# eth-cscs/conflux

Hardware: NVIDIA H100
Metric: LU GFLOP/s (FP64, (2/3)N^3) (higher is better)
Workload: dtype f64

## Files before the change

### conflux_b200/csrc/kernels.h

```cpp
#pragma once
#include <cuda_runtime.h>

#include <cstdint>
#include <memory>

#include "common.cuh"

namespace cflx {

struct GemmArgs {
    int M, N, K;
    const double* AT;
    int64_t ldat;
    const double* B;
    int64_t ldb;
    const double* C;
    int64_t ldc;
    double* D;
    int64_t ldd;
    double alpha, beta;
};
int gemm_tn_setup();
int launch_gemm_tn(const GemmArgs& g, cudaStream_t stream);

struct OzakiWorkspace {
    struct Maps;
    DevBuf<int8_t> planesA;
    DevBuf<int8_t> planesB;
    DevBuf<int> ea;
    DevBuf<int> eb;
    std::unique_ptr<Maps> maps;
    int K = 0, cap_a = 0, cap_b = 0, sms = 0;
    OzakiWorkspace();
    ~OzakiWorkspace();
};
int ozaki_workspace_create(OzakiWorkspace* ws, int max_rows, int max_cols, int K);
int ozaki_split_a(OzakiWorkspace* ws, const double* LT, int64_t ld, int n, cudaStream_t s);
int ozaki_split_b(OzakiWorkspace* ws, const double* U, int64_t ld, int col0, int n, cudaStream_t s);
int wgmma_peak_probe(int n, double* tmacs_out);
int launch_ozaki_gemm(OzakiWorkspace* ws, int M, int N, int row0, int col0, double* C, int64_t ldc, int max_ctas, cudaStream_t s);

struct PanelWorkspace {
    DevBuf<uint2> slot_hdr;
    DevBuf<uint2> slot_rows;
    int epoch;
    int max_ctas;
    int cta_cap;
    DevBuf<unsigned> sk_flags;
    DevBuf<int> sk_ppos;
    DevBuf<unsigned> sk_ticket;
    unsigned sk_epoch, sk_ticket_count;
    int sk_enabled;
};
int panel_workspace_create(PanelWorkspace* ws);
int launch_panel_getrf(double* W, int64_t ldw, int n, int v, int* perm_out, PanelWorkspace* ws, cudaStream_t stream);
int launch_panel_getrf_a00(double* W, int64_t ldw, int n, int v, int* perm_out, double* A00, int* nb_used,
                           PanelWorkspace* ws, cudaStream_t stream);

int launch_extract_panel_T(const double* A, int64_t lda, int64_t row0, int64_t col0, int n, int v, double* PT,
                           int64_t ldp, cudaStream_t stream);
int launch_store_panel_T(double* A, int64_t lda, int64_t row0, int64_t col0, int n, int v, const double* LT,
                         int64_t ldp, cudaStream_t stream);
int launch_gather_winners(const double* PT, int64_t ldp, const int* tags, int n_valid, const int* perm, int v,
                          double* out_vals, int64_t ldo, int* out_tags, int dst0, cudaStream_t stream);
int launch_gather_a00(const double* W, int64_t ldw, const int* perm, int v, int nb, double* A00, double* A00T,
                      cudaStream_t stream);

struct MovePlan {
    int* npiv;
    int* cur_piv;
    int* order;
    int* slot2piv;
    int* early;
    int* late;
    int* nel;
    int* rowsrc;
};
int launch_plan_moves(const int* gpivots, int v, int Px, int pi, int fnpr, int Ml, const int* igri, MovePlan plan,
                      cudaStream_t stream);
int launch_push_phase1(const double* A, int64_t lda, int ncols, int col_lo, MovePlan plan, int v, double* tmp,
                       double* a01raw, int64_t ld01, int c0, cudaStream_t stream);
int launch_push_phase2(double* A, int64_t lda, int ncols, int col_lo, MovePlan plan, int v, cudaStream_t stream);
int launch_push_phase3(double* A, int64_t lda, int ncols, int col_lo, int fnpr, MovePlan plan, int v,
                       const double* tmp, cudaStream_t stream);
int launch_update_gri(int* gri, int* gri_tmp, int* igri, const int* rowsrc, int fnpr, int Ml, int v, int Px,
                      cudaStream_t stream);
int launch_compact_panel(const double* PT, int64_t ldp, double* PT2, int64_t ldp2, const int* rowsrc, int fnpr_old,
                         const int* npiv, int Ml, int v, cudaStream_t stream);
int launch_store_u_rows(double* A, int64_t lda, int fnpr_old, MovePlan plan, const double* U, int64_t ldu, int c0,
                        int ncols, int v, cudaStream_t stream);
int launch_store_diag(double* A, int64_t lda, int fnpr_old, MovePlan plan, const double* A00, int loff, int v,
                      cudaStream_t stream);
int launch_split_factors(const double* F, int64_t ldf, int n, double* LT, double* U, cudaStream_t stream);
int launch_gather_perm_rows(const double* A, int64_t lda, const int* perm, int n, double* out, cudaStream_t stream);
constexpr int SUMSQ_PARTIALS = 1184;
int launch_sumsq(const double* X, int64_t count, double* out, double* partials, cudaStream_t stream);
int launch_sum_partials(const double* partials, int n, double* out, cudaStream_t stream);
int launch_fill(double* p, int64_t n, double val, cudaStream_t stream);
int launch_iota_gri(int* gri, int* igri, int Ml, int v, int Px, int pi, cudaStream_t stream);
int launch_pack_bcast(const double* A00, const int* tags, int v, double* buf, cudaStream_t stream);
int launch_unpack_bcast(const double* buf, int v, double* A00, double* A00T, int* gpivots, cudaStream_t stream);
int launch_record_pivots(const int* gpivots, int v, int* hist, int k, cudaStream_t stream);

int launch_diag_inverses(const double* A00, int v, int nb, double* Uinv, double* LinvT, cudaStream_t stream);
int trsm_right_upper_T(const double* A00, const double* Uinv, int v, int nb, double* PT, double* LT, int64_t ld,
                       int n, cudaStream_t stream);
int trsm_left_lower_unit(const double* A00T, const double* LinvT, int v, int nb, double* R, double* U, int64_t ld,
                         int n, cudaStream_t stream);

size_t potrf_tile_scratch(int v);
int potrf_setup(int v);
int potrf_tile(double* D, double* UT, double* Q, int* info, int col0, int v, cudaStream_t stream, int64_t* launches);
int potrf_block128(double* D, int ldd, double* UT, int ldu, double* Uc, int* info, int col0, cudaStream_t stream);

bool getrf_nopiv_blocked(int v);
size_t getrf_nopiv_scratch(int v, bool blocked);
int launch_getrf_nopiv_tile(const double* Bt, int v, double tiny, double* A, double* AT, const int* tags_in, int* tags_out,
                            int* rec, int col0, bool blocked, double* scratch, cudaStream_t stream, int64_t* launches);
int launch_fixed_locate(const int* rows, int v, int Px, int pi, int fnpr, int n_old, const int* igri, int* pos,
                        cudaStream_t stream);
int launch_fixed_info_operand(int* rec, cudaStream_t stream);

int launch_gather_rows(const double* A, int64_t lda, const int* src_rows, int nrows, int ncols, double* out,
                       cudaStream_t stream);

int launch_gemm_narrow(int M, int N, int K, const double* A, int64_t lda, const double* B, int64_t ldb, const double* C,
                       int64_t ldc, double* D, int64_t ldd, double alpha, double beta, cudaStream_t stream);
int launch_gemm_narrow_tn(int M, int N, int K, const double* AT, int64_t ldat, const double* B, int64_t ldb,
                          const double* C, int64_t ldc, double* D, int64_t ldd, double alpha, double beta,
                          cudaStream_t stream);

enum class ResidMode { NN, TN, SymLower };

}
```

### conflux_b200/csrc/panel.cu

```cuda
#include <cooperative_groups.h>

#include <climits>
#include <cstdlib>

#include "common.cuh"
#include "kernels.h"

namespace cflx {

namespace {
constexpr int PT_THREADS = 256;
constexpr int PT_WARPS = PT_THREADS / 32;
constexpr int PT_LAUNCH = PT_THREADS + 32;
constexpr int PT_ALLWARPS = PT_LAUNCH / 32;
constexpr int MAXG = 132;
constexpr int RPT_LIMIT = 8;

struct PanelArgs {
    double* W;
    int64_t ldw;
    int n, v, nsteps;
    int R, Rpad, G;
    int* perm_out;
    double* A00;
    uint2* slot_hdr;
    uint2* slot_rows;
    int epoch_base;
};

__device__ __forceinline__ void st_ll(uint2* p, unsigned data, unsigned epoch) {
    asm volatile("st.volatile.global.v2.u32 [%0], {%1, %2};" ::"l"(p), "r"(data), "r"(epoch) : "memory");
}
__device__ __forceinline__ uint4 ld_ll2(const uint2* p) {
    uint4 v;
    asm volatile("ld.volatile.global.v4.u32 {%0, %1, %2, %3}, [%4];" : "=r"(v.x), "=r"(v.y), "=r"(v.z), "=r"(v.w) : "l"(p) : "memory");
    return v;
}

struct Cand {
    unsigned long long key;
    int pos;
    int row;
};

__device__ __forceinline__ Cand warp_argmax(Cand c) {
    const unsigned hi = (unsigned)(c.key >> 32), lo = (unsigned)c.key;
    const unsigned m1 = __reduce_max_sync(0xffffffffu, hi);
    bool in = (hi == m1);
    const unsigned m2 = __reduce_max_sync(0xffffffffu, in ? lo : 0u);
    in = in && (lo == m2);
    const unsigned m3 = __reduce_min_sync(0xffffffffu, in ? (unsigned)c.pos : (unsigned)INT_MAX);
    const unsigned ballot = __ballot_sync(0xffffffffu, in && (unsigned)c.pos == m3);
    const int src = __ffs(ballot) - 1;
    Cand r;
    r.key = ((unsigned long long)m1 << 32) | m2;
    r.pos = (int)m3;
    r.row = __shfl_sync(0xffffffffu, c.row, src);
    return r;
}
__device__ __forceinline__ bool better(const Cand& a, const Cand& b) {
    return a.key > b.key || (a.key == b.key && a.pos < b.pos);
}
__device__ __forceinline__ Cand block_argmax(Cand c, unsigned long long* red_key, int* red_pos, int* red_row, int& rb) {
    Cand w = warp_argmax(c);
    const int warp = threadIdx.x >> 5, lane = threadIdx.x & 31;
    const int o = rb * PT_ALLWARPS;
    rb ^= 1;
    if (lane == 0) {
        red_key[o + warp] = w.key;
        red_pos[o + warp] = w.pos;
        red_row[o + warp] = w.row;
    }
    __syncthreads();
    Cand x{0ull, INT_MAX, -1};
    if (lane < PT_ALLWARPS) x = Cand{red_key[o + lane], red_pos[o + lane], red_row[o + lane]};
    return warp_argmax(x);
}

template <int NB, int RPT_MAX>
__global__ void __launch_bounds__(PT_LAUNCH, 1) panel_getrf_kernel(PanelArgs p) {
    extern __shared__ __align__(16) unsigned char smem_raw[];
    double* Ab = reinterpret_cast<double*>(smem_raw);
    double* U12 = Ab + (size_t)NB * p.Rpad;
    double* LU11 = U12 + (size_t)NB * p.v;
    double* prow = LU11 + NB * (NB + 1);
    unsigned long long* red_key = reinterpret_cast<unsigned long long*>(prow + 2 * (NB + 1));
    int* red_pos = reinterpret_cast<int*>(red_key + 2 * PT_ALLWARPS);
    int* red_row = red_pos + 2 * PT_ALLWARPS;
    int* pivrow_blk = red_row + 2 * PT_ALLWARPS;
    int* win_sh = pivrow_blk + NB;
    unsigned char* s_act = reinterpret_cast<unsigned char*>(win_sh + 4);
    int rb = 0;

    const int t = threadIdx.x, warp = t >> 5, lane = t & 31;
    const bool owner = t < PT_THREADS;
    const bool small = p.G <= 32;
    const bool fetcher = warp == (small ? PT_WARPS : 0);
    const int cta = blockIdx.x;
    const int row_base = cta * p.R;
    const int Rloc = max(0, min(p.R, p.n - row_base));
    const int Rpad = p.Rpad, v = p.v;
    double* __restrict__ W = p.W;
    const int64_t ldw = p.ldw;

    int pos[RPT_MAX];
    bool active[RPT_MAX];
#pragma unroll
    for (int q = 0; q < RPT_MAX; ++q) {
        const int lr = t + q * PT_THREADS;
        pos[q] = row_base + lr;
        active[q] = owner && lr < Rloc;
    }
    for (int lr = t; lr < Rpad; lr += PT_LAUNCH) s_act[lr] = lr < Rloc ? 1 : 0;

    for (int jb = 0; jb < p.nsteps; jb += NB) {
        const int nbc = min(NB, v - jb);
        const int nsb = min(nbc, p.nsteps - jb);
        for (int e = t; e < nbc * Rpad; e += PT_LAUNCH) {
            const int c = e / Rpad, lr = e - c * Rpad;
            if (lr < Rloc) Ab[e] = W[(int64_t)(jb + c) * ldw + row_base + lr];
        }
        __syncthreads();

        auto local_candidate = [&](int col) -> Cand {
            Cand c{0ull, INT_MAX, -1};
#pragma unroll
            for (int q = 0; q < RPT_MAX; ++q) {
                const int lr = t + q * PT_THREADS;
                if (active[q]) {
                    Cand o{(unsigned long long)__double_as_longlong(fabs(Ab[col * Rpad + lr])), pos[q], row_base + lr};
                    if (better(o, c)) c = o;
                }
            }
            return block_argmax(c, red_key, red_pos, red_row, rb);
        };
        auto publish = [&](const Cand& mine, int jg, int jprev, const double* pw) {
            const unsigned epoch = (unsigned)(p.epoch_base + jg + 1);
            const int par = jg & 1;
            uint2* myhdr = p.slot_hdr + (size_t)(par * MAXG + cta) * 4;
            if (t < 4) {
                const unsigned w = t == 0 ? (unsigned)mine.key : t == 1 ? (unsigned)(mine.key >> 32)
                                 : t == 2 ? (unsigned)mine.pos : (unsigned)mine.row;
                st_ll(myhdr + t, w, epoch);
            }
            if (t < nbc) {
                double x = 0.0;
                if (mine.row >= 0) {
                    const int lrw = mine.row - row_base;
                    x = Ab[t * Rpad + lrw];
                    if (jprev >= 0 && t > jprev + 1) x = fma(-Ab[jprev * Rpad + lrw], pw[t], x);
                }
                const unsigned long long xb = (unsigned long long)__double_as_longlong(x);
                uint2* myrow = p.slot_rows + (size_t)(par * MAXG + cta) * 64 + 2 * t;
                st_ll(myrow, (unsigned)xb, epoch);
                st_ll(myrow + 1, (unsigned)(xb >> 32), epoch);
            }
        };
        {
            const Cand mine0 = local_candidate(0);
            if (t < 32) __threadfence();
            publish(mine0, jb, -1, nullptr);
        }
        for (int j = 0; j < nsb; ++j) {
            const int jg = jb + j;
            const int par = jg & 1;
            double* pr = prow + par * (NB + 1);
            if (!small || fetcher) {
                const unsigned epoch = (unsigned)(p.epoch_base + jg + 1);
                Cand gc{0ull, INT_MAX, -1};
                for (int g = small ? lane : t; g < p.G; g += small ? 32 : PT_LAUNCH) {
                    const uint2* h = p.slot_hdr + (size_t)(par * MAXG + g) * 4;
                    uint4 a, b;
                    do {
                        a = ld_ll2(h);
                        b = ld_ll2(h + 2);
                    } while (a.y != epoch || a.w != epoch || b.y != epoch || b.w != epoch);
                    Cand o{((unsigned long long)a.z << 32) | a.x, (int)b.x, (int)b.z};
                    if (better(o, gc)) gc = o;
                }
                const Cand w = small ? warp_argmax(gc) : block_argmax(gc, red_key, red_pos, red_row, rb);
                const int wslot = small ? __ffs(__ballot_sync(0xffffffffu, gc.row == w.row)) - 1 : w.row / p.R;
                if (fetcher && lane < nbc) {
                    const uint2* wr = p.slot_rows + (size_t)(par * MAXG + wslot) * 64 + 2 * lane;
                    uint4 a;
                    do {
                        a = ld_ll2(wr);
                    } while (a.y != epoch || a.w != epoch);
                    const double x = __longlong_as_double((long long)(((unsigned long long)a.z << 32) | a.x));
                    pr[lane] = x;
                    LU11[j * (NB + 1) + lane] = x;
                    if (lane == j) pr[NB] = x != 0.0 ? 1.0 / x : 0.0;
                }
                if (fetcher && lane == 0) {
                    win_sh[2 * par] = w.pos;
                    win_sh[2 * par + 1] = w.row;
                }
            }
            __syncthreads();
            Cand win;
            win.key = 0;
            win.pos = win_sh[2 * par];
            win.row = win_sh[2 * par + 1];
            if (t == 0) {
                pivrow_blk[j] = win.row;
                if (cta == 0) p.perm_out[jg] = win.row;
            }
            const double pivot = pr[j];
            const double rinv = pr[NB];
            const bool have_next = (j + 1 < nbc);
            const double pnext = have_next ? pr[j + 1] : 0.0;
            double lq[RPT_MAX];
#pragma unroll
            for (int q = 0; q < RPT_MAX; ++q) {
                const int lr = t + q * PT_THREADS;
                lq[q] = 0.0;
                if (!active[q]) continue;
                if (row_base + lr == win.row) {
                    active[q] = false;
                    s_act[lr] = 0;
                    continue;
                }
                if (pos[q] == jg) pos[q] = win.pos;
                if (pivot != 0.0) {
                    lq[q] = Ab[j * Rpad + lr] * rinv;
                    Ab[j * Rpad + lr] = lq[q];
                }
                if (have_next) Ab[(j + 1) * Rpad + lr] = fma(-lq[q], pnext, Ab[(j + 1) * Rpad + lr]);
            }
            if (j + 1 < nsb) {
                const Cand mine = local_candidate(j + 1);
                publish(mine, jg + 1, j, pr);
                __syncthreads();
            }
            if (owner) {
                double* __restrict__ ab = Ab;
#pragma unroll 4
                for (int c2 = j + 2; c2 < nbc; ++c2) {
                    const double pc = pr[c2];
#pragma unroll
                    for (int q = 0; q < RPT_MAX; ++q) {
                        const int lr = t + q * PT_THREADS;
                        if (active[q]) ab[c2 * Rpad + lr] = fma(-lq[q], pc, ab[c2 * Rpad + lr]);
                    }
                }
            }
        }

        __syncthreads();
        for (int e = t; e < nbc * Rpad; e += PT_LAUNCH) {
            const int c = e / Rpad, lr = e - c * Rpad;
            if (lr < Rloc) W[(int64_t)(jb + c) * ldw + row_base + lr] = Ab[e];
        }
        if (cta == 0 && p.A00 != nullptr) {
            for (int e = t; e < nsb * nbc; e += PT_LAUNCH) {
                const int i = e / nbc, c = e % nbc;
                p.A00[(size_t)(jb + i) * v + jb + c] = LU11[i * (NB + 1) + c];
            }
        }

        const int cstart = jb + nbc;
        const int rem = v - cstart;
        if (rem > 0) {
            __syncthreads();
            __threadfence();
            for (int cc = t; cc < rem; cc += PT_LAUNCH) {
                const double* col = W + (int64_t)(cstart + cc) * ldw;
                double u[NB];
#pragma unroll
                for (int i = 0; i < NB; ++i) u[i] = (i < nsb) ? ld_cg_f64(col + pivrow_blk[i]) : 0.0;
#pragma unroll
                for (int i = 1; i < NB; ++i) {
                    if (i < nsb) {
#pragma unroll
                        for (int s2 = 0; s2 < i; ++s2) u[i] -= LU11[i * (NB + 1) + s2] * u[s2];
                    }
                }
#pragma unroll
                for (int i = 0; i < NB; ++i) U12[i * v + cc] = u[i];
                if (cta == 0 && p.A00 != nullptr) {
#pragma unroll
                    for (int i = 0; i < NB; ++i)
                        if (i < nsb) p.A00[(size_t)(jb + i) * v + cstart + cc] = u[i];
                }
            }
            __syncthreads();
            auto update_row = [&](int lr, int cfirst, int cstep, bool tail) {
                double l[NB];
#pragma unroll
                for (int i = 0; i < NB; ++i) l[i] = (i < nsb) ? Ab[i * Rpad + lr] : 0.0;
                double* wp = W + (int64_t)cstart * ldw + row_base + lr;
                int cc = cfirst;
                double w0 = 0, w1 = 0, w2 = 0, w3 = 0;
                if (cc + 3 < rem) {
                    w0 = wp[(int64_t)cc * ldw];
                    w1 = wp[(int64_t)(cc + 1) * ldw];
                    w2 = wp[(int64_t)(cc + 2) * ldw];
                    w3 = wp[(int64_t)(cc + 3) * ldw];
                }
                for (; cc + 3 < rem; cc += cstep) {
                    double n0 = 0, n1 = 0, n2 = 0, n3 = 0;
                    const int cn = cc + cstep;
                    if (cn + 3 < rem) {
                        n0 = wp[(int64_t)cn * ldw];
                        n1 = wp[(int64_t)(cn + 1) * ldw];
                        n2 = wp[(int64_t)(cn + 2) * ldw];
                        n3 = wp[(int64_t)(cn + 3) * ldw];
                    }
#pragma unroll
                    for (int i = 0; i < NB; ++i) {
                        const double2 ua = *reinterpret_cast<const double2*>(U12 + i * v + cc);
                        const double2 ub = *reinterpret_cast<const double2*>(U12 + i * v + cc + 2);
                        w0 -= l[i] * ua.x;
                        w1 -= l[i] * ua.y;
                        w2 -= l[i] * ub.x;
                        w3 -= l[i] * ub.y;
                    }
                    wp[(int64_t)cc * ldw] = w0;
                    wp[(int64_t)(cc + 1) * ldw] = w1;
                    wp[(int64_t)(cc + 2) * ldw] = w2;
                    wp[(int64_t)(cc + 3) * ldw] = w3;
                    w0 = n0;
                    w1 = n1;
                    w2 = n2;
                    w3 = n3;
                }
                if (tail) {
                    for (int ct = rem & ~3; ct < rem; ++ct) {
                        double x = wp[(int64_t)ct * ldw];
#pragma unroll
                        for (int i = 0; i < NB; ++i) x -= l[i] * U12[i * v + ct];
                        wp[(int64_t)ct * ldw] = x;
                    }
                }
            };
            if (RPT_MAX == 1 && p.R < PT_THREADS) {
                const int nshare = PT_THREADS / p.R;
                const int lr = t % p.R, part = t / p.R;
                if (owner && part < nshare && lr < Rloc && s_act[lr]) update_row(lr, 4 * part, 4 * nshare, part == 0);
            } else {
#pragma unroll 1
                for (int q = 0; q < RPT_MAX; ++q) {
                    const int lr = t + q * PT_THREADS;
                    if (lr >= Rloc || !active[q]) continue;
                    update_row(lr, 0, 4, true);
                }
            }
        }
        __threadfence();
        __syncthreads();
    }
    if (cta == 0)
        for (int i = p.nsteps + t; i < v; i += PT_LAUNCH) p.perm_out[i] = i;
}

constexpr int SK_CB = 16;
struct StackArgs {
    double* W;
    int64_t ldw;
    int n, v;
    int* perm_out;
    int* ppos;
    unsigned* flags;
    unsigned* ticket;
    unsigned ticket_base, epoch;
};
__device__ __forceinline__ unsigned ld_acquire_u32(const unsigned* p) {
    unsigned v;
    asm volatile("ld.acquire.gpu.global.u32 %0, [%1];" : "=r"(v) : "l"(p) : "memory");
    return v;
}
__device__ __forceinline__ void st_release_u32(unsigned* p, unsigned v) {
    asm volatile("st.release.gpu.global.u32 [%0], %1;" ::"l"(p), "r"(v) : "memory");
}
__device__ __forceinline__ void cp_async16(double* smem_dst, const double* gsrc) {
    asm volatile("cp.async.cg.shared.global [%0], [%1], 16;" ::"r"(smem_u32(smem_dst)), "l"(gsrc) : "memory");
}
__device__ __forceinline__ void cp_async_commit() { asm volatile("cp.async.commit_group;" ::: "memory"); }
__device__ __forceinline__ void cp_async_wait_all() { asm volatile("cp.async.wait_all;" ::: "memory"); }

template <int NT>
__global__ void __launch_bounds__(NT, 1) stack_getrf_kernel(StackArgs p) {
    __shared__ double A12s[SK_CB][SK_CB + 1];
    __shared__ double L11s[SK_CB][SK_CB + 1];
    __shared__ double prow[2][SK_CB];
    __shared__ unsigned long long red_key[2][32];
    __shared__ int red_pos[2][32], red_row[2][32];
    __shared__ int pivs[SK_CB], ppos_s[SK_CB];
    __shared__ int s_cta;
    extern __shared__ __align__(16) double Ls[];
    const int t = threadIdx.x, warp = t >> 5, lane = t & 31, nw = blockDim.x >> 5;
    if (t == 0) s_cta = (int)(atomicAdd(p.ticket, 1u) - p.ticket_base);
    __syncthreads();
    const int c = s_cta, c0 = c * SK_CB;
    const bool valid = t < p.n;
    double* __restrict__ W = p.W;
    const int64_t ldw = p.ldw;
    double a[SK_CB];
#pragma unroll
    for (int j = 0; j < SK_CB; ++j) a[j] = valid ? W[(int64_t)(c0 + j) * ldw + t] : 0.0;
    int pos = t;
    int mypiv = -1;

    for (int b = 0; b < c; ++b) {
        if (t == 0)
            while (ld_acquire_u32(p.flags + b) != p.epoch) {}
        __syncthreads();
        if (t < SK_CB) {
            pivs[t] = ld_cg_s32(p.perm_out + b * SK_CB + t);
            ppos_s[t] = ld_cg_s32(p.ppos + b * SK_CB + t);
        }
        {
            const int half = blockDim.x >> 1, q = t % half, h = t / half;
            if (2 * q < p.n) {
                const double* lp = W + (int64_t)(b * SK_CB + 8 * h) * ldw + 2 * q;
#pragma unroll
                for (int k = 0; k < SK_CB / 2; ++k) cp_async16(Ls + (8 * h + k) * NT + 2 * q, lp + (int64_t)k * ldw);
            }
        }
        cp_async_commit();
        __syncthreads();
        int kk = -1;
        if (mypiv < 0) {
#pragma unroll
            for (int k = 0; k < SK_CB; ++k) {
                if (pivs[k] == t) kk = k;
                else if (kk < 0 && pos == b * SK_CB + k) pos = ppos_s[k];
            }
        }
        if (kk >= 0) {
#pragma unroll
            for (int j = 0; j < SK_CB; ++j) A12s[kk][j] = a[j];
#pragma unroll
            for (int k = 0; k < SK_CB; ++k) L11s[kk][k] = ld_cg_f64(W + (int64_t)(b * SK_CB + k) * ldw + t);
        }
        __syncthreads();
        if (t < SK_CB) {
#pragma unroll
            for (int i = 1; i < SK_CB; ++i) {
                double x = A12s[i][t];
#pragma unroll
                for (int s2 = 0; s2 < i; ++s2) x = fma(-L11s[i][s2], A12s[s2][t], x);
                A12s[i][t] = x;
            }
        }
        cp_async_wait_all();
        __syncthreads();
        if (kk >= 0) {
#pragma unroll
            for (int j = 0; j < SK_CB; ++j) a[j] = A12s[kk][j];
            mypiv = b * SK_CB + kk;
        } else if (mypiv < 0 && valid) {
#pragma unroll
            for (int k = 0; k < SK_CB; ++k) {
                const double lk = Ls[k * NT + t];
#pragma unroll
                for (int j = 0; j < SK_CB; ++j) a[j] = fma(-lk, A12s[k][j], a[j]);
            }
        }
    }

#pragma unroll
    for (int j = 0; j < SK_CB; ++j) {
        const int jg = c0 + j, par = j & 1;
        Cand cd{0ull, INT_MAX, -1};
        if (valid && mypiv < 0) cd = Cand{(unsigned long long)__double_as_longlong(fabs(a[j])), pos, t};
        const Cand w1 = warp_argmax(cd);
        if (lane == 0) {
            red_key[par][warp] = w1.key;
            red_pos[par][warp] = w1.pos;
            red_row[par][warp] = w1.row;
        }
        __syncthreads();
        Cand x{0ull, INT_MAX, -1};
        if (lane < nw) x = Cand{red_key[par][lane], red_pos[par][lane], red_row[par][lane]};
        const Cand win = warp_argmax(x);
        if (t == win.row) {
#pragma unroll
            for (int m = 0; m < SK_CB; ++m) prow[par][m] = a[m];
            mypiv = jg;
        }
        if (t == 0) {
            p.perm_out[jg] = win.row;
            p.ppos[jg] = win.pos;
        }
        __syncthreads();
        if (valid && mypiv < 0) {
            if (pos == jg) pos = win.pos;
            const double pivot = prow[par][j];
            const double rinv = pivot != 0.0 ? 1.0 / pivot : 0.0;
            double lq = 0.0;
            if (pivot != 0.0) {
                lq = a[j] * rinv;
                a[j] = lq;
            }
#pragma unroll
            for (int m = j + 1; m < SK_CB; ++m) a[m] = fma(-lq, prow[par][m], a[m]);
        }
    }
    if (valid) {
#pragma unroll
        for (int j = 0; j < SK_CB; ++j) W[(int64_t)(c0 + j) * ldw + t] = a[j];
    }
    __threadfence();
    __syncthreads();
    if (t == 0) st_release_u32(p.flags + c, p.epoch);
}

int launch_stack_getrf(double* W, int64_t ldw, int n, int v, int* perm_out, PanelWorkspace* ws, cudaStream_t stream) {
    StackArgs a{};
    a.W = W;
    a.ldw = ldw;
    a.n = n;
    a.v = v;
    a.perm_out = perm_out;
    a.ppos = ws->sk_ppos;
    a.flags = ws->sk_flags;
    a.ticket = ws->sk_ticket;
    a.ticket_base = ws->sk_ticket_count;
    a.epoch = ++ws->sk_epoch;
    const int C = v / SK_CB;
    ws->sk_ticket_count += (unsigned)C;
    const int threads = (int)round_up(n, 32);
    static PerDeviceMax cfg;
    if (cfg.raise((size_t)SK_CB * 1024 * sizeof(double))) {
        CFLX_CUDA(cudaFuncSetAttribute(stack_getrf_kernel<1024>, cudaFuncAttributeMaxDynamicSharedMemorySize, SK_CB * 1024 * 8));
        CFLX_CUDA(cudaFuncSetAttribute(stack_getrf_kernel<512>, cudaFuncAttributeMaxDynamicSharedMemorySize, SK_CB * 512 * 8));
    }
    if (threads <= 256) stack_getrf_kernel<256><<<C, threads, SK_CB * 256 * sizeof(double), stream>>>(a);
    else if (threads <= 512) stack_getrf_kernel<512><<<C, threads, SK_CB * 512 * sizeof(double), stream>>>(a);
    else stack_getrf_kernel<1024><<<C, threads, SK_CB * 1024 * sizeof(double), stream>>>(a);
    CFLX_CUDA(cudaGetLastError());
    return CFLX_OK;
}

template <int NB>
size_t panel_smem_bytes(int Rpad, int v) {
    return ((size_t)NB * Rpad + (size_t)NB * v + NB * (NB + 1) + 2 * (NB + 1)) * sizeof(double) +
           2 * PT_ALLWARPS * (sizeof(unsigned long long) + 2 * sizeof(int)) +
           (NB + 4) * sizeof(int) + (size_t)Rpad;
}

int panel_nb(int Rpad, int v) {
    for (int nb = 32; nb >= 4; nb /= 2) {
        const long long limit = 222 * 1024 - (8LL * nb * nb + 796LL * nb + 848);
        if ((nb <= v || nb == 4) && (8LL * nb + 1) * Rpad + 8LL * nb * v <= limit) return nb;
    }
    return 0;
}

template <int NB, int RPT>
int launch_nb_rpt(PanelArgs& a, cudaStream_t stream) {
    const size_t smem = panel_smem_bytes<NB>(a.Rpad, a.v);
    void* params[] = {&a};
    static PerDeviceMax cfg;
    if (cfg.raise(smem))
        CFLX_CUDA(cudaFuncSetAttribute(panel_getrf_kernel<NB, RPT>, cudaFuncAttributeMaxDynamicSharedMemorySize, (int)smem));
    CFLX_CUDA(cudaLaunchCooperativeKernel((void*)panel_getrf_kernel<NB, RPT>, dim3(a.G), dim3(PT_LAUNCH), params, smem, stream));
    return CFLX_OK;
}
template <int NB>
int launch_nb(PanelArgs& a, cudaStream_t stream) {
    const int rpt = (a.R + PT_THREADS - 1) / PT_THREADS;
    if (rpt <= 1) return launch_nb_rpt<NB, 1>(a, stream);
    if (rpt <= 2) return launch_nb_rpt<NB, 2>(a, stream);
    if (rpt <= 4) return launch_nb_rpt<NB, 4>(a, stream);
    return launch_nb_rpt<NB, 8>(a, stream);
}
}


int panel_workspace_create(PanelWorkspace* ws) {
    int dev = 0, sms = 0;
    CFLX_CUDA(cudaGetDevice(&dev));
    CFLX_CUDA(cudaDeviceGetAttribute(&sms, cudaDevAttrMultiProcessorCount, dev));
    ws->max_ctas = sms < MAXG ? sms : MAXG;
    ws->epoch = 1;
    ws->cta_cap = 0;
    CFLX_TRY(ws->slot_hdr.alloc_exact(2 * MAXG * 4));
    CFLX_TRY(ws->slot_rows.alloc_exact(2 * MAXG * 64));
    CFLX_CUDA(cudaMemset(ws->slot_hdr, 0, sizeof(uint2) * 2 * MAXG * 4));
    CFLX_CUDA(cudaMemset(ws->slot_rows, 0, sizeof(uint2) * 2 * MAXG * 64));
    CFLX_TRY(ws->sk_flags.alloc_exact(1024));
    CFLX_TRY(ws->sk_ppos.alloc_exact(16384));
    CFLX_TRY(ws->sk_ticket.alloc_exact(1));
    CFLX_CUDA(cudaMemset(ws->sk_flags, 0, sizeof(unsigned) * 1024));
    CFLX_CUDA(cudaMemset(ws->sk_ticket, 0, sizeof(unsigned)));
    ws->sk_epoch = 0;
    ws->sk_ticket_count = 0;
    {
        const char* e = getenv("CFLX_STACK_KERNEL");
        ws->sk_enabled = e ? atoi(e) : 1;
    }
    return CFLX_OK;
}

int launch_panel_getrf_a00(double* W, int64_t ldw, int n, int v, int* perm_out, double* A00, int* nb_used,
                           PanelWorkspace* ws, cudaStream_t stream) {
    if (v <= 0 || n < 0) return CFLX_ERR_ARG;
    if (ws->sk_enabled && n >= v && n <= 1024 && v % SK_CB == 0 && v <= 16384 && ldw % 2 == 0 &&
        (reinterpret_cast<uintptr_t>(W) & 15) == 0) {
        if (nb_used) *nb_used = 0;
        return launch_stack_getrf(W, ldw, n, v, perm_out, ws, stream);
    }
    PanelArgs a{};
    a.W = W;
    a.ldw = ldw;
    a.n = n;
    a.v = v;
    a.nsteps = n < v ? n : v;
    int G = (n + 31) / 32;
    if (G < 1) G = 1;
    if (G > ws->max_ctas) G = ws->max_ctas;
    if (ws->cta_cap > 0 && G > ws->cta_cap) {
        G = ws->cta_cap;
        const int need = (n + RPT_LIMIT * PT_THREADS - 1) / (RPT_LIMIT * PT_THREADS);
        if (G < need) G = need < ws->max_ctas ? need : ws->max_ctas;
    }
    int R = (n + G - 1) / G;
    R = (int)round_up(R > 0 ? R : 1, 32);
    G = n > 0 ? (n + R - 1) / R : 1;
    if (R > RPT_LIMIT * PT_THREADS) {
        set_last_error("panel_getrf: n=%d rows exceed the %d-row capacity (%d CTAs x %d rows)", n,
                       ws->max_ctas * RPT_LIMIT * PT_THREADS, ws->max_ctas, RPT_LIMIT * PT_THREADS);
        return CFLX_ERR_UNSUPPORTED;
    }
    a.R = R;
    a.Rpad = R;
    a.G = G;
    a.perm_out = perm_out;
    a.A00 = A00;
    a.slot_hdr = ws->slot_hdr;
    a.slot_rows = ws->slot_rows;
    a.epoch_base = ws->epoch;
    ws->epoch += v + 2 + (v & 1);
    const int nb = panel_nb(a.Rpad, v);
    if (nb == 0) {
        set_last_error("panel_getrf: v=%d with %d rows per CTA exceeds the shared-memory budget of the inner block", v,
                       a.Rpad);
        return CFLX_ERR_UNSUPPORTED;
    }
    if (nb_used) *nb_used = nb;
    switch (nb) {
        case 32: return launch_nb<32>(a, stream);
        case 16: return launch_nb<16>(a, stream);
        case 8: return launch_nb<8>(a, stream);
        default: return launch_nb<4>(a, stream);
    }
}

int launch_panel_getrf(double* W, int64_t ldw, int n, int v, int* perm_out, PanelWorkspace* ws, cudaStream_t stream) {
    return launch_panel_getrf_a00(W, ldw, n, v, perm_out, nullptr, nullptr, ws, stream);
}

}
```

Measured before the change: 25190.

## Defer panel trailing update into next block's pivot steps, add fast argmax path

Adds an optional deferred trailing-update mode to the panel getrf kernel. It copies the L block into shared memory and spreads the remaining column updates across the pivot-search steps of the next block, so the update overlaps the latency-bound pivot phase. It also adds a warp-reduction shortcut for when a single lane holds the max key, pads Rpad by one to reduce shared-memory bank conflicts, and moves the A00 U-row writes out of the inner loop. Deferral sits behind an env var that is off by default and costs extra shared memory.

```diff
diff --git a/conflux_b200/csrc/kernels.h b/conflux_b200/csrc/kernels.h
--- a/conflux_b200/csrc/kernels.h
+++ b/conflux_b200/csrc/kernels.h
@@ -46,6 +46,8 @@
     int epoch;
     int max_ctas;
     int cta_cap;
+    int smem_max;
+    int defer_enabled;
     DevBuf<unsigned> sk_flags;
     DevBuf<int> sk_ppos;
     DevBuf<unsigned> sk_ticket;
diff --git a/conflux_b200/csrc/panel.cu b/conflux_b200/csrc/panel.cu
--- a/conflux_b200/csrc/panel.cu
+++ b/conflux_b200/csrc/panel.cu
@@ -21,6 +21,7 @@
     int64_t ldw;
     int n, v, nsteps;
     int R, Rpad, G;
+    int defer;
     int* perm_out;
     double* A00;
     uint2* slot_hdr;
@@ -47,6 +48,15 @@
     const unsigned hi = (unsigned)(c.key >> 32), lo = (unsigned)c.key;
     const unsigned m1 = __reduce_max_sync(0xffffffffu, hi);
     bool in = (hi == m1);
+    const unsigned bhi = __ballot_sync(0xffffffffu, in);
+    if (__popc(bhi) == 1) {
+        const int src = __ffs(bhi) - 1;
+        Cand r;
+        r.key = ((unsigned long long)m1 << 32) | __shfl_sync(0xffffffffu, lo, src);
+        r.pos = __shfl_sync(0xffffffffu, c.pos, src);
+        r.row = __shfl_sync(0xffffffffu, c.row, src);
+        return r;
+    }
     const unsigned m2 = __reduce_max_sync(0xffffffffu, in ? lo : 0u);
     in = in && (lo == m2);
     const unsigned m3 = __reduce_min_sync(0xffffffffu, in ? (unsigned)c.pos : (unsigned)INT_MAX);
@@ -81,7 +91,8 @@
 __global__ void __launch_bounds__(PT_LAUNCH, 1) panel_getrf_kernel(PanelArgs p) {
     extern __shared__ __align__(16) unsigned char smem_raw[];
     double* Ab = reinterpret_cast<double*>(smem_raw);
-    double* U12 = Ab + (size_t)NB * p.Rpad;
+    double* Lb = Ab + (size_t)NB * p.Rpad;
+    double* U12 = Lb + (p.defer ? (size_t)NB * p.Rpad : 0);
     double* LU11 = U12 + (size_t)NB * p.v;
     double* prow = LU11 + NB * (NB + 1);
     unsigned long long* red_key = reinterpret_cast<unsigned long long*>(prow + 2 * (NB + 1));
@@ -113,6 +124,67 @@
     }
     for (int lr = t; lr < Rpad; lr += PT_LAUNCH) s_act[lr] = lr < Rloc ? 1 : 0;
 
+    const bool share = RPT_MAX == 1 && p.R < PT_THREADS;
+    auto update_mask = [&]() -> unsigned {
+        unsigned m = 0;
+        if (share) {
+            const int lr = t % p.R, part = t / p.R;
+            if (owner && part < PT_THREADS / p.R && lr < Rloc && s_act[lr]) m = 1u;
+        } else {
+#pragma unroll
+            for (int q = 0; q < RPT_MAX; ++q)
+                if (t + q * PT_THREADS < Rloc && active[q]) m |= 1u << q;
+        }
+        return m;
+    };
+    int dcs = 0;
+    unsigned dmask = 0;
+    auto deferred_row = [&](int lr, int cfirst, int cstep, int clim, bool tail) {
+        double* wp = W + (int64_t)dcs * ldw + row_base + lr;
+        const int rem_ = v - dcs;
+        double l[NB];
+#pragma unroll
+        for (int i = 0; i < NB; ++i) l[i] = Lb[i * Rpad + lr];
+#pragma unroll 1
+        for (int cc = cfirst; cc + 3 < clim; cc += cstep) {
+            double w0 = wp[(int64_t)cc * ldw], w1 = wp[(int64_t)(cc + 1) * ldw];
+            double w2 = wp[(int64_t)(cc + 2) * ldw], w3 = wp[(int64_t)(cc + 3) * ldw];
+#pragma unroll
+            for (int i = 0; i < NB; ++i) {
+                const double li = l[i];
+                const double2 ua = *reinterpret_cast<const double2*>(U12 + i * v + cc);
+                const double2 ub = *reinterpret_cast<const double2*>(U12 + i * v + cc + 2);
+                w0 -= li * ua.x;
+                w1 -= li * ua.y;
+                w2 -= li * ub.x;
+                w3 -= li * ub.y;
+            }
+            wp[(int64_t)cc * ldw] = w0;
+            wp[(int64_t)(cc + 1) * ldw] = w1;
+            wp[(int64_t)(cc + 2) * ldw] = w2;
+            wp[(int64_t)(cc + 3) * ldw] = w3;
+        }
+        if (tail) {
+            for (int ct = rem_ & ~3; ct < rem_; ++ct) {
+                double x = wp[(int64_t)ct * ldw];
+#pragma unroll
+                for (int i = 0; i < NB; ++i) x -= l[i] * U12[i * v + ct];
+                wp[(int64_t)ct * ldw] = x;
+            }
+        }
+    };
+    auto run_deferred = [&](int g0, int g1, bool last) {
+        const int c0 = NB + 4 * g0, c1 = NB + 4 * g1;
+        if (share) {
+            const int part = t / p.R;
+            if (dmask) deferred_row(t % p.R, c0 + 4 * part, 4 * (PT_THREADS / p.R), c1, last && part == 0);
+        } else {
+#pragma unroll 1
+            for (int q = 0; q < RPT_MAX; ++q)
+                if ((dmask >> q) & 1u) deferred_row(t + q * PT_THREADS, c0, 4, c1, last);
+        }
+    };
+
     for (int jb = 0; jb < p.nsteps; jb += NB) {
         const int nbc = min(NB, v - jb);
         const int nsb = min(nbc, p.nsteps - jb);
@@ -121,6 +193,9 @@
             if (lr < Rloc) Ab[e] = W[(int64_t)(jb + c) * ldw + row_base + lr];
         }
         __syncthreads();
+
+        const int dslots = dcs > 0 ? nsb - 2 : 0;
+        const int dgroups = (v - dcs - NB) >> 2;
 
         auto local_candidate = [&](int col) -> Cand {
             Cand c{0ull, INT_MAX, -1};
@@ -229,6 +304,7 @@
             }
             if (j + 1 < nsb) {
                 const Cand mine = local_candidate(j + 1);
+                if (dslots > 0 && j + 2 == nsb && t < 32) __threadfence();
                 publish(mine, jg + 1, j, pr);
                 __syncthreads();
             }
@@ -243,13 +319,22 @@
                         if (active[q]) ab[c2 * Rpad + lr] = fma(-lq[q], pc, ab[c2 * Rpad + lr]);
                     }
                 }
-            }
-        }
-
+                if (j < dslots) {
+                    run_deferred(j * dgroups / dslots, (j + 1) * dgroups / dslots, j + 1 == dslots);
+                    if (j + 1 == dslots) __threadfence();
+                }
+            }
+        }
+        dcs = 0;
+
+        const int cstart = jb + nbc;
+        const int rem = v - cstart;
+        const bool defer = p.defer && rem > NB && p.nsteps - (jb + NB) >= 3;
         __syncthreads();
         for (int e = t; e < nbc * Rpad; e += PT_LAUNCH) {
             const int c = e / Rpad, lr = e - c * Rpad;
             if (lr < Rloc) W[(int64_t)(jb + c) * ldw + row_base + lr] = Ab[e];
+            if (defer) Lb[e] = Ab[e];
         }
         if (cta == 0 && p.A00 != nullptr) {
             for (int e = t; e < nsb * nbc; e += PT_LAUNCH) {
@@ -258,8 +343,6 @@
             }
         }
 
-        const int cstart = jb + nbc;
-        const int rem = v - cstart;
         if (rem > 0) {
             __syncthreads();
             __threadfence();
@@ -277,13 +360,15 @@
                 }
 #pragma unroll
                 for (int i = 0; i < NB; ++i) U12[i * v + cc] = u[i];
-                if (cta == 0 && p.A00 != nullptr) {
-#pragma unroll
-                    for (int i = 0; i < NB; ++i)
-                        if (i < nsb) p.A00[(size_t)(jb + i) * v + cstart + cc] = u[i];
-                }
             }
             __syncthreads();
+            if (cta == 0 && p.A00 != nullptr) {
+                for (int e = t; e < nsb * rem; e += PT_LAUNCH) {
+                    const int i = e / rem, cc = e - i * rem;
+                    p.A00[(size_t)(jb + i) * v + cstart + cc] = U12[i * v + cc];
+                }
+            }
+            const int remv = defer ? NB : rem;
             auto update_row = [&](int lr, int cfirst, int cstep, bool tail) {
                 double l[NB];
 #pragma unroll
@@ -291,16 +376,16 @@
                 double* wp = W + (int64_t)cstart * ldw + row_base + lr;
                 int cc = cfirst;
                 double w0 = 0, w1 = 0, w2 = 0, w3 = 0;
-                if (cc + 3 < rem) {
+                if (cc + 3 < remv) {
                     w0 = wp[(int64_t)cc * ldw];
                     w1 = wp[(int64_t)(cc + 1) * ldw];
                     w2 = wp[(int64_t)(cc + 2) * ldw];
                     w3 = wp[(int64_t)(cc + 3) * ldw];
                 }
-                for (; cc + 3 < rem; cc += cstep) {
+                for (; cc + 3 < remv; cc += cstep) {
                     double n0 = 0, n1 = 0, n2 = 0, n3 = 0;
                     const int cn = cc + cstep;
-                    if (cn + 3 < rem) {
+                    if (cn + 3 < remv) {
                         n0 = wp[(int64_t)cn * ldw];
                         n1 = wp[(int64_t)(cn + 1) * ldw];
                         n2 = wp[(int64_t)(cn + 2) * ldw];
@@ -325,7 +410,7 @@
                     w3 = n3;
                 }
                 if (tail) {
-                    for (int ct = rem & ~3; ct < rem; ++ct) {
+                    for (int ct = remv & ~3; ct < remv; ++ct) {
                         double x = wp[(int64_t)ct * ldw];
 #pragma unroll
                         for (int i = 0; i < NB; ++i) x -= l[i] * U12[i * v + ct];
@@ -333,17 +418,18 @@
                     }
                 }
             };
-            if (RPT_MAX == 1 && p.R < PT_THREADS) {
-                const int nshare = PT_THREADS / p.R;
+            const unsigned mask = update_mask();
+            if (share) {
                 const int lr = t % p.R, part = t / p.R;
-                if (owner && part < nshare && lr < Rloc && s_act[lr]) update_row(lr, 4 * part, 4 * nshare, part == 0);
+                if (mask) update_row(lr, 4 * part, 4 * (PT_THREADS / p.R), part == 0);
             } else {
 #pragma unroll 1
-                for (int q = 0; q < RPT_MAX; ++q) {
-                    const int lr = t + q * PT_THREADS;
-                    if (lr >= Rloc || !active[q]) continue;
-                    update_row(lr, 0, 4, true);
-                }
+                for (int q = 0; q < RPT_MAX; ++q)
+                    if ((mask >> q) & 1u) update_row(t + q * PT_THREADS, 0, 4, true);
+            }
+            if (defer) {
+                dmask = mask;
+                dcs = cstart;
             }
         }
         __threadfence();
@@ -534,23 +620,24 @@
 }
 
 template <int NB>
-size_t panel_smem_bytes(int Rpad, int v) {
-    return ((size_t)NB * Rpad + (size_t)NB * v + NB * (NB + 1) + 2 * (NB + 1)) * sizeof(double) +
+size_t panel_smem_bytes(int Rpad, int v, bool defer) {
+    return ((size_t)NB * Rpad * (defer ? 2 : 1) + (size_t)NB * v + NB * (NB + 1) + 2 * (NB + 1)) * sizeof(double) +
            2 * PT_ALLWARPS * (sizeof(unsigned long long) + 2 * sizeof(int)) +
            (NB + 4) * sizeof(int) + (size_t)Rpad;
 }
 
-int panel_nb(int Rpad, int v) {
+int panel_nb(int R, int v) {
     for (int nb = 32; nb >= 4; nb /= 2) {
         const long long limit = 222 * 1024 - (8LL * nb * nb + 796LL * nb + 848);
-        if ((nb <= v || nb == 4) && (8LL * nb + 1) * Rpad + 8LL * nb * v <= limit) return nb;
+        if ((nb <= v || nb == 4) && (8LL * nb + 1) * R + 8LL * nb * v <= limit) return nb;
     }
     return 0;
 }
 
 template <int NB, int RPT>
-int launch_nb_rpt(PanelArgs& a, cudaStream_t stream) {
-    const size_t smem = panel_smem_bytes<NB>(a.Rpad, a.v);
+int launch_nb_rpt(PanelArgs& a, size_t smem_max, cudaStream_t stream) {
+    if (a.defer && panel_smem_bytes<NB>(a.Rpad, a.v, true) > smem_max) a.defer = 0;
+    const size_t smem = panel_smem_bytes<NB>(a.Rpad, a.v, a.defer != 0);
     void* params[] = {&a};
     static PerDeviceMax cfg;
     if (cfg.raise(smem))
@@ -559,12 +646,12 @@
     return CFLX_OK;
 }
 template <int NB>
-int launch_nb(PanelArgs& a, cudaStream_t stream) {
+int launch_nb(PanelArgs& a, size_t smem_max, cudaStream_t stream) {
     const int rpt = (a.R + PT_THREADS - 1) / PT_THREADS;
-    if (rpt <= 1) return launch_nb_rpt<NB, 1>(a, stream);
-    if (rpt <= 2) return launch_nb_rpt<NB, 2>(a, stream);
-    if (rpt <= 4) return launch_nb_rpt<NB, 4>(a, stream);
-    return launch_nb_rpt<NB, 8>(a, stream);
+    if (rpt <= 1) return launch_nb_rpt<NB, 1>(a, smem_max, stream);
+    if (rpt <= 2) return launch_nb_rpt<NB, 2>(a, smem_max, stream);
+    if (rpt <= 4) return launch_nb_rpt<NB, 4>(a, smem_max, stream);
+    return launch_nb_rpt<NB, 8>(a, smem_max, stream);
 }
 }
 
@@ -574,6 +661,7 @@
     CFLX_CUDA(cudaGetDevice(&dev));
     CFLX_CUDA(cudaDeviceGetAttribute(&sms, cudaDevAttrMultiProcessorCount, dev));
     ws->max_ctas = sms < MAXG ? sms : MAXG;
+    CFLX_CUDA(cudaDeviceGetAttribute(&ws->smem_max, cudaDevAttrMaxSharedMemoryPerBlockOptin, dev));
     ws->epoch = 1;
     ws->cta_cap = 0;
     CFLX_TRY(ws->slot_hdr.alloc_exact(2 * MAXG * 4));
@@ -591,6 +679,10 @@
         const char* e = getenv("CFLX_STACK_KERNEL");
         ws->sk_enabled = e ? atoi(e) : 1;
     }
+    {
+        const char* e = getenv("CFLX_PANEL_DEFER");
+        ws->defer_enabled = e ? atoi(e) : 0;
+    }
     return CFLX_OK;
 }
 
@@ -625,26 +717,26 @@
         return CFLX_ERR_UNSUPPORTED;
     }
     a.R = R;
-    a.Rpad = R;
+    a.Rpad = R + 1;
     a.G = G;
+    a.defer = ws->defer_enabled && G <= 32;
     a.perm_out = perm_out;
     a.A00 = A00;
     a.slot_hdr = ws->slot_hdr;
     a.slot_rows = ws->slot_rows;
     a.epoch_base = ws->epoch;
     ws->epoch += v + 2 + (v & 1);
-    const int nb = panel_nb(a.Rpad, v);
+    const int nb = panel_nb(R, v);
     if (nb == 0) {
-        set_last_error("panel_getrf: v=%d with %d rows per CTA exceeds the shared-memory budget of the inner block", v,
-                       a.Rpad);
+        set_last_error("panel_getrf: v=%d with %d rows per CTA exceeds the shared-memory budget of the inner block", v, R);
         return CFLX_ERR_UNSUPPORTED;
     }
     if (nb_used) *nb_used = nb;
     switch (nb) {
-        case 32: return launch_nb<32>(a, stream);
-        case 16: return launch_nb<16>(a, stream);
-        case 8: return launch_nb<8>(a, stream);
-        default: return launch_nb<4>(a, stream);
+        case 32: return launch_nb<32>(a, (size_t)ws->smem_max, stream);
+        case 16: return launch_nb<16>(a, (size_t)ws->smem_max, stream);
+        case 8: return launch_nb<8>(a, (size_t)ws->smem_max, stream);
+        default: return launch_nb<4>(a, (size_t)ws->smem_max, stream);
     }
 }
 
```

Result: no change. 25310 (median of 6 runs) (+0.5%).
